# supranational/sppark

Measured on AMD Instinct MI355X. Metric: MSM points/sec (BLS12-381 G1, 2^26 points), higher is better.
Workload: dtype u32

## Files before the change

### sppark_amd/csrc/ec/xyzzx_dev.hpp

```cpp
#pragma once
#include "../ff/montx_dev.hpp"
#include "xyzz_dev.hpp"

namespace sppark_amd {

template<class FP> struct field_is_internal { static constexpr bool value = false; };
template<class P, int LB> struct field_is_internal<montx_dev<P, LB>> { static constexpr bool value = true; };
template<class FP> struct field_is_montx { static constexpr bool value = false; };
template<class P, int LB> struct field_is_montx<montx_dev<P, LB>> { static constexpr bool value = true; };

template<class P, int LB> struct affine_loader<montx_dev<P, LB>> {
    typedef montx_dev<P, LB> F;
    static constexpr unsigned RAW = 2 * F::NL * 4;
    static constexpr unsigned STRIDE = RAW <= 64 ? 64 : RAW <= 128 ? 128 : ((RAW + 15) / 16) * 16;
    struct raw_t {
        u32 w[(RAW + 15) / 16 * 4];
        SPPARK_DEVFN void landed() const
        {
#if defined(__HIP_DEVICE_COMPILE__)
            #pragma unroll
            for (unsigned i = 0; i < (RAW + 15) / 16 * 4; i++) asm volatile("" :: "v"(w[i]));
#endif
        }
    };
// ... 15 lines not shown
    }
    template<bool FLAGGED>
    SPPARK_DEVFN static affine_dev<F> load(const unsigned char* base, size_t idx, unsigned)
    {   return decode(load_raw(base, idx));   }
    template<bool FLAGGED>
    SPPARK_DEVFN static void convert(unsigned char* dst, const unsigned char* src, size_t idx, unsigned stride)
    {
        typedef mont_dev<P> S;
        u32 wx[S::N], wy[S::N];
        bool inf;
        if (!FLAGGED && (S::N % 2) == 0 && (stride & 15) == 0 && ((size_t)src & 15) == 0) {
            const uint4* q = reinterpret_cast<const uint4*>(src + idx * (size_t)stride);
            u32 w[2 * S::N];
            #pragma unroll
            for (int i = 0; i < S::N / 2; i++) { uint4 v = q[i]; w[4*i] = v.x; w[4*i+1] = v.y; w[4*i+2] = v.z; w[4*i+3] = v.w; }
            u32 any = 0;
            #pragma unroll
            for (int i = 0; i < S::N; i++) { wx[i] = w[i]; wy[i] = w[S::N + i]; any |= w[i] | w[S::N + i]; }
            inf = any == 0;
        } else {
            affine_dev<S> p = affine_loader<S>::template load<FLAGGED>(src, idx, stride);
            p.X.to_wire(wx); p.Y.to_wire(wy);
            inf = p.inf;
        }
        F x = F::from_std(wx), y = F::from_std(wy);
        u32 w[STRIDE / 4] = {};
        x.to_wire(w); y.to_wire(w + F::NL);
        if (inf) w[F::NL - 1] |= 0x80000000u;
        uint4* q = reinterpret_cast<uint4*>(dst + idx * (size_t)STRIDE);
        #pragma unroll
        for (unsigned i = 0; i < STRIDE / 16; i++) q[i] = make_uint4(w[4*i], w[4*i+1], w[4*i+2], w[4*i+3]);
    }
};

template<class P, int LB> struct xyzz_dev<montx_dev<P, LB>> {
    typedef montx_dev<P, LB> F;
    F X, Y, ZZZ, ZZ;
    static constexpr bool TIGHT = F::TIGHT;
    static constexpr int BX = TIGHT ? 1 : 6;
    static constexpr int BX2 = TIGHT ? 1 : 4;
    SPPARK_DEVFN static F keep_x(const F& x3) { if constexpr (TIGHT) return x3.norm(); else return x3; }
    SPPARK_DEVFN static F minus_y(const F& y) { if constexpr (TIGHT) return F::template neg<4, 2>(y); else return F::template neg<6, 4>(y); }

    SPPARK_DEVFN bool is_inf() const { return ZZ.limbs_all_zero(); }
    SPPARK_DEVFN void set_inf() { X = F::zero(); Y = F::zero(); ZZZ = F::zero(); ZZ = F::zero(); }

    SPPARK_DEVFN void set(const affine_dev<F>& p, bool negate)
    {
        if (p.inf) { set_inf(); return; }
        X = p.X; Y = negate ? F::template neg<3>(p.Y) : p.Y;
        ZZZ = F::one(); ZZ = F::one();
    }

    SPPARK_DEVFN void madd(const affine_dev<F>& p, bool negate)
    {
        if (p.inf) return;
        if (is_inf()) { set(p, negate); return; }

        F U2, S2;
        F::template mul2<true, true>(U2, S2, p.X, ZZ, p.Y, ZZZ);
        if (negate) S2 = F::template neg<3>(S2);
        F Pd = F::template sub<11, BX>(U2, X).norm();
        F Rd;
        if constexpr (TIGHT) Rd = F::template sub<4, 2>(S2, Y).norm(); else Rd = F::template sub<6, 4>(S2, Y).norm();

        if (!Pd.template is_zero_mod<13>()) {
            F PP, RR, PPP, Q;
            F::sqr2(PP, RR, Pd, Rd);
            F::template mul2<true, false>(PPP, Q, Pd, PP, X, PP);
            F T   = PPP + Q + Q;
            F X3  = keep_x(F::template sub<8, 3>(RR, T));
            F D   = F::template sub<11, BX>(Q, X3);
            F nY  = minus_y(Y);
            Y   = F::mul_add(D, Rd, nY, PPP);
            F::template mul2<true, true>(ZZ, ZZZ, ZZ, PP, ZZZ, PPP);
            X = X3;
        } else if (Rd.template is_zero_mod<9>()) {
            F y2 = negate ? F::template neg<3>(p.Y).norm() : p.Y;
            dbl_affine(p.X, y2);
        } else {
            set_inf();
        }
    }

    SPPARK_DEVFN void add(const xyzz_dev& q)
    {
        if (q.is_inf()) return;
        if (is_inf()) { *this = q; return; }

        F U1 = X * q.ZZ;
        F S1 = Y * q.ZZZ;
        F U2 = q.X * ZZ;
        F S2 = q.Y * ZZZ;
        F Pd = F::template sub<3>(U2, U1).norm();
        F Rd = F::template sub<3>(S2, S1).norm();

        if (!Pd.template is_zero_mod<5>()) {
            F PP  = Pd.sqr();
            F PPP = Pd * PP;
            F Q   = U1 * PP;
            F T   = PPP + Q + Q;
            F X3  = keep_x(F::template sub<8, 3>(Rd.sqr(), T));
            F D   = F::template sub<11, BX>(Q, X3);
            Y   = F::mul_add(D, Rd, F::template neg<3>(S1), PPP);
            ZZ  = (ZZ * PP) * q.ZZ;
            ZZZ = (ZZZ * PPP) * q.ZZZ;
            X = X3;
        } else if (Rd.template is_zero_mod<5>()) {
            xyzz_dev t = *this;
            dbl_outlined(t);
            *this = t;
        } else {
            set_inf();
        }
    }

    SPPARK_DEVFN void add_pairs(const xyzz_dev& q)
    {
        if (q.is_inf()) return;
        if (is_inf()) { *this = q; return; }
        F U1, S1, U2, S2;
        F::mul2(U1, S1, X, q.ZZ, Y, q.ZZZ);
        F::mul2(U2, S2, q.X, ZZ, q.Y, ZZZ);
        F Pd = F::template sub<3>(U2, U1).norm();
        F Rd = F::template sub<3>(S2, S1).norm();
        if (!Pd.template is_zero_mod<5>()) {
            F PP, RR, PPP, Q, t0, t1;
            F::sqr2(PP, RR, Pd, Rd);
            F::template mul2<true, true>(PPP, Q, Pd, PP, U1, PP);
            F T   = PPP + Q + Q;
            F X3  = keep_x(F::template sub<8, 3>(RR, T));
            F D   = F::template sub<11, BX>(Q, X3);
            Y   = F::mul_add(D, Rd, F::template neg<3>(S1), PPP);
            F::template mul2<true, true>(t0, t1, ZZ, PP, ZZZ, PPP);
// ... 102 lines not shown
```

### sppark_amd/csrc/ff/montx_blocks.hpp

```cpp
#pragma once
namespace sppark_amd {
#define MX_MAD(A, x, y) "v_mad_u64_u32 %[" #A "], vcc, %[" #x "], %[" #y "], %[" #A "]\n\t"
#define MX_SHR(A)       "v_lshrrev_b64 %[" #A "], %[LB], %[" #A "]\n\t"
#define MX_ADD(A, B)    "v_lshl_add_u64 %[" #A "], %[" #A "], 0, %[" #B "]\n\t"
#define MX_V(name, e)   [name] "v"(e)
#define MX_S(name, j)   [name] "s"(pl<F, j>)
#define MX_ASM(text, outs, ...) asm(text : outs : __VA_ARGS__, [LB] "n"(F::LIMB_BITS) : "vcc")
#define MX_ASM0(text, outs)     asm(text : outs : [LB] "n"(F::LIMB_BITS) : "vcc")
#define MX_ACC1 [A] "+v"(A)
#define MX_ACC2 [A0] "+v"(A0), [A1] "+v"(A1)
#define MX_ACCS [A] "+v"(A), [B] "+v"(B)
#define MX_I(j) (LO + j)
#define MX_J(j) (K - LO - j)
#define MX_MAX_TERMS 14
#define MX_T_AB1_1 MX_MAD(A, x0_0, y0_0)
#define MX_T_AB1_2 MX_T_AB1_1 MX_MAD(A, x0_1, y0_1)
#define MX_T_AB1_3 MX_T_AB1_2 MX_MAD(A, x0_2, y0_2)
#define MX_T_AB1_4 MX_T_AB1_3 MX_MAD(A, x0_3, y0_3)
#define MX_T_AB1_5 MX_T_AB1_4 MX_MAD(A, x0_4, y0_4)
#define MX_T_AB1_6 MX_T_AB1_5 MX_MAD(A, x0_5, y0_5)
#define MX_T_AB1_7 MX_T_AB1_6 MX_MAD(A, x0_6, y0_6)
#define MX_T_AB1_8 MX_T_AB1_7 MX_MAD(A, x0_7, y0_7)
#define MX_T_AB1_9 MX_T_AB1_8 MX_MAD(A, x0_8, y0_8)
#define MX_T_AB1_10 MX_T_AB1_9 MX_MAD(A, x0_9, y0_9)
#define MX_T_AB1_11 MX_T_AB1_10 MX_MAD(A, x0_10, y0_10)
#define MX_T_AB1_12 MX_T_AB1_11 MX_MAD(A, x0_11, y0_11)
#define MX_T_AB1_13 MX_T_AB1_12 MX_MAD(A, x0_12, y0_12)
#define MX_T_AB1_14 MX_T_AB1_13 MX_MAD(A, x0_13, y0_13)
#define MX_O_AB1_1 MX_V(x0_0, o.x0(MX_I(0), MX_J(0))), MX_V(y0_0, o.y0(MX_I(0), MX_J(0)))
#define MX_O_AB1_2 MX_O_AB1_1, MX_V(x0_1, o.x0(MX_I(1), MX_J(1))), MX_V(y0_1, o.y0(MX_I(1), MX_J(1)))
#define MX_O_AB1_3 MX_O_AB1_2, MX_V(x0_2, o.x0(MX_I(2), MX_J(2))), MX_V(y0_2, o.y0(MX_I(2), MX_J(2)))
#define MX_O_AB1_4 MX_O_AB1_3, MX_V(x0_3, o.x0(MX_I(3), MX_J(3))), MX_V(y0_3, o.y0(MX_I(3), MX_J(3)))
#define MX_O_AB1_5 MX_O_AB1_4, MX_V(x0_4, o.x0(MX_I(4), MX_J(4))), MX_V(y0_4, o.y0(MX_I(4), MX_J(4)))
#define MX_O_AB1_6 MX_O_AB1_5, MX_V(x0_5, o.x0(MX_I(5), MX_J(5))), MX_V(y0_5, o.y0(MX_I(5), MX_J(5)))
#define MX_O_AB1_7 MX_O_AB1_6, MX_V(x0_6, o.x0(MX_I(6), MX_J(6))), MX_V(y0_6, o.y0(MX_I(6), MX_J(6)))
#define MX_O_AB1_8 MX_O_AB1_7, MX_V(x0_7, o.x0(MX_I(7), MX_J(7))), MX_V(y0_7, o.y0(MX_I(7), MX_J(7)))
#define MX_O_AB1_9 MX_O_AB1_8, MX_V(x0_8, o.x0(MX_I(8), MX_J(8))), MX_V(y0_8, o.y0(MX_I(8), MX_J(8)))
#define MX_O_AB1_10 MX_O_AB1_9, MX_V(x0_9, o.x0(MX_I(9), MX_J(9))), MX_V(y0_9, o.y0(MX_I(9), MX_J(9)))
#define MX_O_AB1_11 MX_O_AB1_10, MX_V(x0_10, o.x0(MX_I(10), MX_J(10))), MX_V(y0_10, o.y0(MX_I(10), MX_J(10)))
#define MX_O_AB1_12 MX_O_AB1_11, MX_V(x0_11, o.x0(MX_I(11), MX_J(11))), MX_V(y0_11, o.y0(MX_I(11), MX_J(11)))
#define MX_O_AB1_13 MX_O_AB1_12, MX_V(x0_12, o.x0(MX_I(12), MX_J(12))), MX_V(y0_12, o.y0(MX_I(12), MX_J(12)))
#define MX_O_AB1_14 MX_O_AB1_13, MX_V(x0_13, o.x0(MX_I(13), MX_J(13))), MX_V(y0_13, o.y0(MX_I(13), MX_J(13)))
#define MX_T_MP1_1 MX_MAD(A, m0_0, p_0)
#define MX_T_MP1_2 MX_T_MP1_1 MX_MAD(A, m0_1, p_1)
#define MX_T_MP1_3 MX_T_MP1_2 MX_MAD(A, m0_2, p_2)
#define MX_T_MP1_4 MX_T_MP1_3 MX_MAD(A, m0_3, p_3)
#define MX_T_MP1_5 MX_T_MP1_4 MX_MAD(A, m0_4, p_4)
#define MX_T_MP1_6 MX_T_MP1_5 MX_MAD(A, m0_5, p_5)
#define MX_T_MP1_7 MX_T_MP1_6 MX_MAD(A, m0_6, p_6)
#define MX_T_MP1_8 MX_T_MP1_7 MX_MAD(A, m0_7, p_7)
#define MX_T_MP1_9 MX_T_MP1_8 MX_MAD(A, m0_8, p_8)
#define MX_T_MP1_10 MX_T_MP1_9 MX_MAD(A, m0_9, p_9)
#define MX_T_MP1_11 MX_T_MP1_10 MX_MAD(A, m0_10, p_10)
#define MX_T_MP1_12 MX_T_MP1_11 MX_MAD(A, m0_11, p_11)
#define MX_T_MP1_13 MX_T_MP1_12 MX_MAD(A, m0_12, p_12)
#define MX_T_MP1_14 MX_T_MP1_13 MX_MAD(A, m0_13, p_13)
#define MX_O_MP1_1 MX_V(m0_0, o.m0(MX_I(0))), MX_S(p_0, MX_J(0))
// ... 235 lines not shown
        else if constexpr (!CLOSE && NAB == 12 && NMP == 12) MX_ASM(MX_SHR(A0) MX_SHR(A1) MX_T_AB2_12(A0, A1) MX_T_MP2_12, MX_ACC2, MX_O_AB2_12, MX_O_MP2_12);
        else static_assert(K < 0, "no block of this shape");
#else
        if constexpr (CLOSE) { A0 += (u64)o.m0(K - 1) * F::mod_limb(0); A1 += (u64)o.m1(K - 1) * F::mod_limb(0); }
        if constexpr (K > 0) { A0 >>= F::LIMB_BITS; A1 >>= F::LIMB_BITS; }
        for (int j = 0; j < NAB; j++) { A0 += (u64)o.x0(MX_I(j), MX_J(j)) * o.y0(MX_I(j), MX_J(j)); A1 += (u64)o.x1(MX_I(j), MX_J(j)) * o.y1(MX_I(j), MX_J(j)); }
        for (int j = 0; j < NMP; j++) { A0 += (u64)o.m0(MX_I(j)) * F::mod_limb(MX_J(j)); A1 += (u64)o.m1(MX_I(j)) * F::mod_limb(MX_J(j)); }
#endif
    }
    template<class F, int K, class OPS> SPPARK_DEVFN static void col_sum(u64& A, const OPS& o)
    {
        MX_SHAPE;
        [[maybe_unused]] u64 B = 0;
#if defined(__HIP_DEVICE_COMPILE__)
        if constexpr (LAST) MX_ASM0(MX_SHR(A), MX_ACC1);
        else if constexpr (K == 0) { static_assert(NAB == 1 && NMP == 0, "shape"); asm(MX_T_AB2_1(A, B) MX_ADD(A, B) : MX_ACCS : MX_O_AB2_1 : "vcc"); }
        else if constexpr (CLOSE && NAB == 2 && NMP == 1) MX_ASM(MX_MAD(A, mc0, pc) MX_SHR(A) MX_T_AB2_2(A, B) MX_T_MPS_1 MX_ADD(A, B), MX_ACCS, MX_V(mc0, o.m0(K - 1)), MX_S(pc, 0), MX_O_AB2_2, MX_O_MP1_1);
        else if constexpr (CLOSE && NAB == 3 && NMP == 2) MX_ASM(MX_MAD(A, mc0, pc) MX_SHR(A) MX_T_AB2_3(A, B) MX_T_MPS_2 MX_ADD(A, B), MX_ACCS, MX_V(mc0, o.m0(K - 1)), MX_S(pc, 0), MX_O_AB2_3, MX_O_MP1_2);
        else if constexpr (CLOSE && NAB == 4 && NMP == 3) MX_ASM(MX_MAD(A, mc0, pc) MX_SHR(A) MX_T_AB2_4(A, B) MX_T_MPS_3 MX_ADD(A, B), MX_ACCS, MX_V(mc0, o.m0(K - 1)), MX_S(pc, 0), MX_O_AB2_4, MX_O_MP1_3);
        else if constexpr (CLOSE && NAB == 5 && NMP == 4) MX_ASM(MX_MAD(A, mc0, pc) MX_SHR(A) MX_T_AB2_5(A, B) MX_T_MPS_4 MX_ADD(A, B), MX_ACCS, MX_V(mc0, o.m0(K - 1)), MX_S(pc, 0), MX_O_AB2_5, MX_O_MP1_4);
        else if constexpr (CLOSE && NAB == 6 && NMP == 5) MX_ASM(MX_MAD(A, mc0, pc) MX_SHR(A) MX_T_AB2_6(A, B) MX_T_MPS_5 MX_ADD(A, B), MX_ACCS, MX_V(mc0, o.m0(K - 1)), MX_S(pc, 0), MX_O_AB2_6, MX_O_MP1_5);
        else if constexpr (CLOSE && NAB == 7 && NMP == 6) MX_ASM(MX_MAD(A, mc0, pc) MX_SHR(A) MX_T_AB2_7(A, B) MX_T_MPS_6 MX_ADD(A, B), MX_ACCS, MX_V(mc0, o.m0(K - 1)), MX_S(pc, 0), MX_O_AB2_7, MX_O_MP1_6);
        else if constexpr (CLOSE && NAB == 8 && NMP == 7) MX_ASM(MX_MAD(A, mc0, pc) MX_SHR(A) MX_T_AB2_8(A, B) MX_T_MPS_7 MX_ADD(A, B), MX_ACCS, MX_V(mc0, o.m0(K - 1)), MX_S(pc, 0), MX_O_AB2_8, MX_O_MP1_7);
        else if constexpr (CLOSE && NAB == 8 && NMP == 8) MX_ASM(MX_MAD(A, mc0, pc) MX_SHR(A) MX_T_AB2_8(A, B) MX_T_MPS_8 MX_ADD(A, B), MX_ACCS, MX_V(mc0, o.m0(K - 1)), MX_S(pc, 0), MX_O_AB2_8, MX_O_MP1_8);
        else if constexpr (CLOSE && NAB == 9 && NMP == 8) MX_ASM(MX_MAD(A, mc0, pc) MX_SHR(A) MX_T_AB2_9(A, B) MX_T_MPS_8 MX_ADD(A, B), MX_ACCS, MX_V(mc0, o.m0(K - 1)), MX_S(pc, 0), MX_O_AB2_9, MX_O_MP1_8);
        else if constexpr (CLOSE && NAB == 9 && NMP == 9) MX_ASM(MX_MAD(A, mc0, pc) MX_SHR(A) MX_T_AB2_9(A, B) MX_T_MPS_9 MX_ADD(A, B), MX_ACCS, MX_V(mc0, o.m0(K - 1)), MX_S(pc, 0), MX_O_AB2_9, MX_O_MP1_9);
        else if constexpr (CLOSE && NAB == 10 && NMP == 9) MX_ASM(MX_MAD(A, mc0, pc) MX_SHR(A) MX_T_AB2_10(A, B) MX_T_MPS_9 MX_ADD(A, B), MX_ACCS, MX_V(mc0, o.m0(K - 1)), MX_S(pc, 0), MX_O_AB2_10, MX_O_MP1_9);
        else if constexpr (CLOSE && NAB == 11 && NMP == 10) MX_ASM(MX_MAD(A, mc0, pc) MX_SHR(A) MX_T_AB2_11(A, B) MX_T_MPS_10 MX_ADD(A, B), MX_ACCS, MX_V(mc0, o.m0(K - 1)), MX_S(pc, 0), MX_O_AB2_11, MX_O_MP1_10);
        else if constexpr (CLOSE && NAB == 12 && NMP == 11) MX_ASM(MX_MAD(A, mc0, pc) MX_SHR(A) MX_T_AB2_12(A, B) MX_T_MPS_11 MX_ADD(A, B), MX_ACCS, MX_V(mc0, o.m0(K - 1)), MX_S(pc, 0), MX_O_AB2_12, MX_O_MP1_11);
        else if constexpr (CLOSE && NAB == 13 && NMP == 12) MX_ASM(MX_MAD(A, mc0, pc) MX_SHR(A) MX_T_AB2_13(A, B) MX_T_MPS_12 MX_ADD(A, B), MX_ACCS, MX_V(mc0, o.m0(K - 1)), MX_S(pc, 0), MX_O_AB2_13, MX_O_MP1_12);
        else if constexpr (CLOSE && NAB == 13 && NMP == 13) MX_ASM(MX_MAD(A, mc0, pc) MX_SHR(A) MX_T_AB2_13(A, B) MX_T_MPS_13 MX_ADD(A, B), MX_ACCS, MX_V(mc0, o.m0(K - 1)), MX_S(pc, 0), MX_O_AB2_13, MX_O_MP1_13);
        else if constexpr (CLOSE && NAB == 14 && NMP == 13) MX_ASM(MX_MAD(A, mc0, pc) MX_SHR(A) MX_T_AB2_14(A, B) MX_T_MPS_13 MX_ADD(A, B), MX_ACCS, MX_V(mc0, o.m0(K - 1)), MX_S(pc, 0), MX_O_AB2_14, MX_O_MP1_13);
        else if constexpr (!CLOSE && NAB == 1 && NMP == 1) MX_ASM(MX_SHR(A) MX_T_AB2_1(A, B) MX_T_MPS_1 MX_ADD(A, B), MX_ACCS, MX_O_AB2_1, MX_O_MP1_1);
        else if constexpr (!CLOSE && NAB == 2 && NMP == 2) MX_ASM(MX_SHR(A) MX_T_AB2_2(A, B) MX_T_MPS_2 MX_ADD(A, B), MX_ACCS, MX_O_AB2_2, MX_O_MP1_2);
        else if constexpr (!CLOSE && NAB == 3 && NMP == 3) MX_ASM(MX_SHR(A) MX_T_AB2_3(A, B) MX_T_MPS_3 MX_ADD(A, B), MX_ACCS, MX_O_AB2_3, MX_O_MP1_3);
        else if constexpr (!CLOSE && NAB == 4 && NMP == 4) MX_ASM(MX_SHR(A) MX_T_AB2_4(A, B) MX_T_MPS_4 MX_ADD(A, B), MX_ACCS, MX_O_AB2_4, MX_O_MP1_4);
        else if constexpr (!CLOSE && NAB == 5 && NMP == 5) MX_ASM(MX_SHR(A) MX_T_AB2_5(A, B) MX_T_MPS_5 MX_ADD(A, B), MX_ACCS, MX_O_AB2_5, MX_O_MP1_5);
        else if constexpr (!CLOSE && NAB == 6 && NMP == 6) MX_ASM(MX_SHR(A) MX_T_AB2_6(A, B) MX_T_MPS_6 MX_ADD(A, B), MX_ACCS, MX_O_AB2_6, MX_O_MP1_6);
        else if constexpr (!CLOSE && NAB == 7 && NMP == 7) MX_ASM(MX_SHR(A) MX_T_AB2_7(A, B) MX_T_MPS_7 MX_ADD(A, B), MX_ACCS, MX_O_AB2_7, MX_O_MP1_7);
        else if constexpr (!CLOSE && NAB == 8 && NMP == 8) MX_ASM(MX_SHR(A) MX_T_AB2_8(A, B) MX_T_MPS_8 MX_ADD(A, B), MX_ACCS, MX_O_AB2_8, MX_O_MP1_8);
        else if constexpr (!CLOSE && NAB == 9 && NMP == 9) MX_ASM(MX_SHR(A) MX_T_AB2_9(A, B) MX_T_MPS_9 MX_ADD(A, B), MX_ACCS, MX_O_AB2_9, MX_O_MP1_9);
        else if constexpr (!CLOSE && NAB == 10 && NMP == 10) MX_ASM(MX_SHR(A) MX_T_AB2_10(A, B) MX_T_MPS_10 MX_ADD(A, B), MX_ACCS, MX_O_AB2_10, MX_O_MP1_10);
        else if constexpr (!CLOSE && NAB == 11 && NMP == 11) MX_ASM(MX_SHR(A) MX_T_AB2_11(A, B) MX_T_MPS_11 MX_ADD(A, B), MX_ACCS, MX_O_AB2_11, MX_O_MP1_11);
        else if constexpr (!CLOSE && NAB == 12 && NMP == 12) MX_ASM(MX_SHR(A) MX_T_AB2_12(A, B) MX_T_MPS_12 MX_ADD(A, B), MX_ACCS, MX_O_AB2_12, MX_O_MP1_12);
        else static_assert(K < 0, "no block of this shape");
#else
        if constexpr (CLOSE) A += (u64)o.m0(K - 1) * F::mod_limb(0);
        if constexpr (K > 0) A >>= F::LIMB_BITS;
        for (int j = 0; j < NAB; j++) { A += (u64)o.x0(MX_I(j), MX_J(j)) * o.y0(MX_I(j), MX_J(j)); B += (u64)o.x1(MX_I(j), MX_J(j)) * o.y1(MX_I(j), MX_J(j)); }
        for (int j = 0; j < NMP; j++) (j & 1 ? B : A) += (u64)o.m0(MX_I(j)) * F::mod_limb(MX_J(j));
        A += B;
#endif
    }
};
#undef MX_MAD
#undef MX_SHR
#undef MX_ADD
#undef MX_V
#undef MX_S
#undef MX_ASM
#undef MX_ASM0
#undef MX_ACC1
#undef MX_ACC2
#undef MX_ACCS
#undef MX_I
#undef MX_J
#undef MX_SHAPE
#undef MX_O_AB1_1
#undef MX_O_AB1_10
#undef MX_O_AB1_11
#undef MX_O_AB1_12
#undef MX_O_AB1_13
#undef MX_O_AB1_14
#undef MX_O_AB1_2
#undef MX_O_AB1_3
#undef MX_O_AB1_4
#undef MX_O_AB1_5
#undef MX_O_AB1_6
#undef MX_O_AB1_7
#undef MX_O_AB1_8
#undef MX_O_AB1_9
#undef MX_O_AB2_1
#undef MX_O_AB2_10
#undef MX_O_AB2_11
#undef MX_O_AB2_12
#undef MX_O_AB2_13
#undef MX_O_AB2_14
#undef MX_O_AB2_2
#undef MX_O_AB2_3
#undef MX_O_AB2_4
#undef MX_O_AB2_5
#undef MX_O_AB2_6
#undef MX_O_AB2_7
#undef MX_O_AB2_8
#undef MX_O_AB2_9
#undef MX_O_MP1_1
#undef MX_O_MP1_10
#undef MX_O_MP1_11
#undef MX_O_MP1_12
#undef MX_O_MP1_13
#undef MX_O_MP1_14
#undef MX_O_MP1_2
#undef MX_O_MP1_3
#undef MX_O_MP1_4
#undef MX_O_MP1_5
#undef MX_O_MP1_6
#undef MX_O_MP1_7
#undef MX_O_MP1_8
#undef MX_O_MP1_9
#undef MX_O_MP2_1
// ... 86 lines not shown
```

### sppark_amd/csrc/ff/montx_dev.hpp

```cpp
#pragma once
#include "mont_dev.hpp"
#include "montx_blocks.hpp"
#include <utility>

namespace sppark_amd {


#if defined(SPPARK_HOST_EMULATION) && defined(SPPARK_TRACK_BOUNDS)
extern "C" void sppark_bound_violation(const char* what, double got, double limit);
#endif
template<class P, int LB> struct montx_dev {
    static constexpr int NW = P::N;
    static constexpr int HEAD = LB <= 28 ? 8 : 6;
    static constexpr int NL = (P::NBITS + HEAD + LB - 1) / LB;
    static constexpr int CAP = 1 << (32 - LB);
    static constexpr int FAT_L = 1 << (31 - LB);
    static constexpr bool TIGHT = LB > 28;
    static constexpr bool FAT_M_OK = (double)NL * (4294967296.0 * (double)(1ull << LB) + (double)(1ull << LB) * (double)(1ull << LB))
                                     + 68719476736.0 < 18446744073709551616.0;
    static constexpr int MA_A0 = TIGHT ? 3 : FAT_L, MA_A1 = TIGHT ? 3 : 6;
    static constexpr int SQR_L = TIGHT ? 2 : 4;
    static constexpr int N = NL;
    static constexpr int LIMB_BITS = LB;
    typedef montx_blocks blk;
// ... 169 lines not shown
    }

    SPPARK_DEVFN static montx_dev from_wire(const u32* w)
    {   montx_dev r; for (int j = 0; j < NL; j++) r.l[j] = w[j]; return r;   }
    SPPARK_DEVFN void to_wire(u32* w) const { for (int j = 0; j < NL; j++) w[j] = l[j]; }

    SPPARK_DEVFN static montx_dev zero() { montx_dev r; for (int j = 0; j < NL; j++) r.l[j] = 0; SPPARK_BND(r.bnd_set(0.0, 0.0);) return r; }
    SPPARK_DEVFN bool limbs_all_zero() const
    {   u32 acc = l[0]; for (int j = 1; j < NL; j++) acc |= l[j]; return acc == 0;   }

    SPPARK_DEVFN montx_dev norm() const
    {
        montx_dev r; u32 c = 0;
        #pragma unroll
        for (int j = 0; j < NL - 1; j++) { u32 v = l[j] + c; r.l[j] = v & MASK; c = v >> LB; }
        r.l[NL - 1] = l[NL - 1] + c;
        SPPARK_BND(bnd_known("norm: operand"); bnd(bl <= (double)(CAP - 1), "norm: limbs", bl, (double)(CAP - 1)); r.bnd_set(bv, bl < 1.0 ? bl : 1.0);)
        return r;
    }

    SPPARK_DEVFN friend montx_dev operator+(const montx_dev& a, const montx_dev& b)
    {
        montx_dev r;
        #pragma unroll
        for (int j = 0; j < NL; j++) r.l[j] = a.l[j] + b.l[j];
        SPPARK_BND(a.bnd_known("+: left"); b.bnd_known("+: right"); r.bnd_set(a.bv + b.bv, a.bl + b.bl); bnd(r.bl < (double)CAP, "+: limbs wrap", r.bl, (double)CAP);)
        return r;
    }

    template<int K, int B = 1> SPPARK_DEVFN static montx_dev sub(const montx_dev& a, const montx_dev& b)
    {
        montx_dev r;
        #pragma unroll
        for (int j = 0; j < NL; j++) r.l[j] = a.l[j] + (fat_tab<K, B>::T.l[j] - b.l[j]);
        SPPARK_BND(a.bnd_known("sub: minuend"); b.bnd_known("sub: subtrahend");
                   bnd(b.bv <= (double)(K - 1), "sub<K>: subtrahend < (K-1) p", b.bv, (double)(K - 1));
                   bnd(b.bl <= (double)B, "sub<K,B>: subtrahend's limbs <= B 2^LB", b.bl, (double)B);
                   r.bnd_set(a.bv + (double)K, a.bl + (double)(B + 1));
                   bnd(r.bl < (double)CAP, "sub: limbs wrap", r.bl, (double)CAP);)
        return r;
    }
    template<int K, int B = 1> SPPARK_DEVFN static montx_dev neg(const montx_dev& b)
    {
        montx_dev r;
        #pragma unroll
        for (int j = 0; j < NL; j++) r.l[j] = fat_tab<K, B>::T.l[j] - b.l[j];
        SPPARK_BND(b.bnd_known("neg: operand");
                   bnd(b.bv <= (double)(K - 1), "neg<K>: operand < (K-1) p", b.bv, (double)(K - 1));
                   bnd(b.bl <= (double)B, "neg<K,B>: operand's limbs <= B 2^LB", b.bl, (double)B);
                   r.bnd_set((double)K, (double)(B + 1));)
        return r;
    }


    SPPARK_DEVFN friend montx_dev operator*(const montx_dev& a, const montx_dev& b)
    {
        constexpr u32 PINV = P::M0 & MASK;
        u32 m[NL];
        montx_dev r;
        u64 A = 0;
        for_columns([&] SPPARK_COLUMN(kc, k)
            blk::template col1<montx_dev, k>(A, blk::mul_ops{a.l, b.l, nullptr, nullptr, m, nullptr});
            if constexpr (k < NL) m[k] = ((u32)A * PINV) & MASK;
            else        r.l[k - NL] = (u32)A & MASK;
        });
        SPPARK_BND(a.bnd_known("*: left"); b.bnd_known("*: right");
                   bnd(b.bl <= 1.0, "*: right operand normalised", b.bl, 1.0);
                   bnd(a.bl <= FAT_LEFT + 1e-6, "*: left operand's limbs < 2^31", a.bl, FAT_LEFT);
                   r.bnd_set(a.bv * b.bv / rho() + 1.0, 1.0);)
        return r;
    }
    template<bool FAT_M> SPPARK_DEVFN static u32 quotient_digit(u64 A, int k)
    {
        constexpr u32 PINV = P::M0 & MASK;
        if (FAT_M && FAT_M_OK && k < NL - 1) return (u32)A * (u32)P::M0;
        return ((u32)A * PINV) & MASK;
    }

    template<bool NORM0 = false, bool NORM1 = false>
    SPPARK_DEVFN static void mul2(montx_dev& r0, montx_dev& r1,
                                  const montx_dev& a0, const montx_dev& b0,
                                  const montx_dev& a1, const montx_dev& b1)
    {
        u32 m0[NL], m1[NL];
        u64 A0 = 0, A1 = 0;
        for_columns([&] SPPARK_COLUMN(kc, k)
            blk::template col2<montx_dev, k>(A0, A1, blk::mul_ops{a0.l, b0.l, a1.l, b1.l, m0, m1});
            if constexpr (k < NL) { m0[k] = quotient_digit<NORM0>(A0, k); m1[k] = quotient_digit<NORM1>(A1, k); }
            else        { r0.l[k - NL] = (u32)A0 & MASK; r1.l[k - NL] = (u32)A1 & MASK; }
        });
        SPPARK_BND(a0.bnd_known("mul2: a0"); b0.bnd_known("mul2: b0"); a1.bnd_known("mul2: a1"); b1.bnd_known("mul2: b1");
                   bnd(b0.bl <= 1.0 && b1.bl <= 1.0, "mul2: right operands normalised", b0.bl > b1.bl ? b0.bl : b1.bl, 1.0);
                   bnd(a0.bl <= (NORM0 ? 1.0 : FAT_LEFT) + 1e-6, NORM0 ? "mul2<NORM0>: a0 normalised" : "mul2: a0's limbs < 2^31", a0.bl, NORM0 ? 1.0 : FAT_LEFT);
                   bnd(a1.bl <= (NORM1 ? 1.0 : FAT_LEFT) + 1e-6, NORM1 ? "mul2<NORM1>: a1 normalised" : "mul2: a1's limbs < 2^31", a1.bl, NORM1 ? 1.0 : FAT_LEFT);
                   r0.bnd_set(a0.bv * b0.bv / rho() + 1.0 + (NORM0 ? 1e-6 : 0.0), 1.0);
                   r1.bnd_set(a1.bv * b1.bv / rho() + 1.0 + (NORM1 ? 1e-6 : 0.0), 1.0);)
    }
    SPPARK_DEVFN static montx_dev mul_add(const montx_dev& a0, const montx_dev& b0,
                                          const montx_dev& a1, const montx_dev& b1)
    {
        static_assert((double)NL * ((double)MA_A0 + (double)MA_A1 + 1.0) * (double)(1ull << LB) * (double)(1ull << LB) + 68719476736.0
                      < 18446744073709551616.0, "a column of two products must fit the 64-bit accumulator");
        constexpr u32 PINV = P::M0 & MASK;
        u32 m[NL];
        montx_dev r;
        u64 A = 0;
        for_columns([&] SPPARK_COLUMN(kc, k)
            blk::template col_sum<montx_dev, k>(A, blk::mul_ops{a0.l, b0.l, a1.l, b1.l, m, nullptr});
            if constexpr (k < NL) m[k] = ((u32)A * PINV) & MASK;
            else        r.l[k - NL] = (u32)A & MASK;
        });
        SPPARK_BND(a0.bnd_known("mul_add: a0"); b0.bnd_known("mul_add: b0"); a1.bnd_known("mul_add: a1"); b1.bnd_known("mul_add: b1");
                   bnd(b0.bl <= 1.0 && b1.bl <= 1.0, "mul_add: right operands normalised", b0.bl > b1.bl ? b0.bl : b1.bl, 1.0);
                   bnd(a0.bl <= (double)MA_A0 + 1e-6, "mul_add: a0's limbs <= MA_A0 2^LB", a0.bl, (double)MA_A0);
                   bnd(a1.bl <= (double)MA_A1, "mul_add: a1's limbs <= MA_A1 2^LB", a1.bl, (double)MA_A1);
                   r.bnd_set((a0.bv * b0.bv + a1.bv * b1.bv) / rho() + 1.0, 1.0);)
        return r;
    }

    SPPARK_DEVFN static void sqr2(montx_dev& r0, montx_dev& r1, const montx_dev& a0, const montx_dev& a1)
    {
        u32 m0[NL], m1[NL], d0[NL], d1[NL];
        #pragma unroll
        for (int j = 0; j < NL; j++) { d0[j] = a0.l[j] << 1; d1[j] = a1.l[j] << 1; }
        u64 A0 = 0, A1 = 0;
        for_columns([&] SPPARK_COLUMN(kc, k)
            blk::template col2<montx_dev, k>(A0, A1, blk::sqr_ops{a0.l, d0, a1.l, d1, m0, m1});
            if constexpr (k < NL) { m0[k] = quotient_digit<true>(A0, k); m1[k] = quotient_digit<true>(A1, k); }
            else        { r0.l[k - NL] = (u32)A0 & MASK; r1.l[k - NL] = (u32)A1 & MASK; }
        });
        SPPARK_BND(a0.bnd_known("sqr2: a0"); a1.bnd_known("sqr2: a1");
                   bnd(a0.bl <= 1.0 && a1.bl <= 1.0, "sqr2: operands normalised", a0.bl > a1.bl ? a0.bl : a1.bl, 1.0);
                   r0.bnd_set(a0.bv * a0.bv / rho() + 1.0 + 1e-6, 1.0); r1.bnd_set(a1.bv * a1.bv / rho() + 1.0 + 1e-6, 1.0);)
    }

    SPPARK_DEVFN montx_dev sqr() const
    {
        static_assert(((double)(NL / 2) * 2.0 * SQR_L * SQR_L + (double)(SQR_L * SQR_L) + (double)NL) * (double)(1ull << LB) * (double)(1ull << LB)
                      + 68719476736.0 < 18446744073709551616.0, "a column of a square of limbs <= SQR_L 2^LB must fit the 64-bit accumulator");
        constexpr u32 PINV = P::M0 & MASK;
        u32 m[NL], d[NL];
        #pragma unroll
        for (int j = 0; j < NL; j++) d[j] = l[j] << 1;
        montx_dev r;
        u64 A = 0;
        for_columns([&] SPPARK_COLUMN(kc, k)
            blk::template col1<montx_dev, k>(A, blk::sqr_ops{l, d, nullptr, nullptr, m, nullptr});
            if constexpr (k < NL) m[k] = ((u32)A * PINV) & MASK;
            else        r.l[k - NL] = (u32)A & MASK;
        });
        SPPARK_BND(bnd_known("sqr: operand"); bnd(bl <= (double)SQR_L, "sqr: limbs <= SQR_L 2^LB", bl, (double)SQR_L); r.bnd_set(bv * bv / rho() + 1.0, 1.0);)
        return r;
    }

    SPPARK_DEVFN montx_dev inverse() const
    {
        montx_dev r = one();
        bool started = false;
        #pragma unroll 1
        for (int w = NW - 1; w >= 0; w--) {
            u32 e = 0, borrow = 2;
            for (int k = 0; k <= w; k++) { e = P::MOD[k] - borrow; borrow = P::MOD[k] < borrow ? 1u : 0u; }
            #pragma unroll 1
            for (int b = 31; b >= 0; b--) {
                if (started) r = r.sqr();
                if ((e >> b) & 1u) { r = started ? r * *this : *this; started = true; }
            }
        }
        return r;
    }

    template<int KMAX> SPPARK_DEVFN bool is_zero_mod() const
    {
        SPPARK_BND(bnd_known("is_zero_mod: operand"); bnd(bl <= 1.0, "is_zero_mod: normalised", bl, 1.0);
                   bnd(bv <= (double)KMAX, "is_zero_mod<KMAX>: value < KMAX p", bv, (double)KMAX);)
        bool maybe = false;
        #pragma unroll
        for (int kk = 0; kk < KMAX; kk++) maybe |= (l[0] == multiples_tab<KMAX>::T.l[kk][0]);
        if (!maybe) return false;
        bool hit = false;
        #pragma unroll 1
        for (int k = 0; k < KMAX; k++) {
            u32 diff = 0;
            #pragma unroll
            for (int j = 0; j < NL; j++) diff |= multiples_tab<KMAX>::T.l[k][j] ^ l[j];
            hit |= diff == 0;
        }
        return hit;
    }
};

}
```

### sppark_amd/csrc/msm/msm_kernels.hpp

```cpp
#pragma once
#include "../ec/xyzz_dev.hpp"
#include "../ec/xyzzx_dev.hpp"

namespace sppark_amd {

static constexpr u32 KEY_NONE = 0xffffffffu;


__host__ __device__ inline unsigned window_len(unsigned w, unsigned nwins, unsigned nbits)
{   return nbits / nwins + (w < nbits % nwins ? 1u : 0u);   }

template<class LimbFn>
SPPARK_DEVFN void recode_digits(u32* digits, size_t n, size_t i, LimbFn limb, bool flip,
                                unsigned nwins, unsigned nbits, unsigned w_begin = 0, unsigned w_count = ~0u)
{
    u32 carry = 0;
    const unsigned w_end = w_count > nwins - w_begin ? nwins : w_begin + w_count;
    for (unsigned w = 0, bit = 0; w < w_end; w++) {
        const unsigned len = window_len(w, nwins, nbits);
        const u32 half = 1u << (len - 1), full = 1u << len, mask = full - 1;
        const unsigned li = bit >> 5, sh = bit & 31;
        bit += len;
        u64 two = limb(li) | ((u64)limb(li + 1) << 32);
        u32 d = ((u32)(two >> sh) & mask) + carry;
// ... 23 lines not shown
    flip = bw != 0;
    return FR::select(flip, neg, s);
}

template<class FR>
__global__ __launch_bounds__(256)
void k_breakdown(u32* __restrict__ digits, const u32* __restrict__ scalars,
                 unsigned n, unsigned nwins, unsigned nbits, int mont, unsigned w_begin, unsigned w_count)
{
    constexpr int N = FR::N;
    __shared__ u32 limbs[N + 2][256];
    const unsigned tid = threadIdx.x;
    for (unsigned i = blockIdx.x * 256 + tid; i < n; i += gridDim.x * 256) {
        bool flip;
        FR s = load_scalar_abs<FR>(scalars, i, mont, flip);
        #pragma unroll
        for (int k = 0; k < N; k++) limbs[k][tid] = s.v[k];
        limbs[N][tid] = 0; limbs[N + 1][tid] = 0;
        recode_digits(digits, n, i, [&](unsigned k) { return limbs[k][tid]; }, flip, nwins, nbits, w_begin, w_count);
    }
}

template<class FP, bool ON> struct gather_raw { struct type {}; };
template<class FP> struct gather_raw<FP, true> { typedef typename affine_loader<FP>::raw_t type; };

template<class FP, bool FLAGGED>
SPPARK_DEVFN void accumulate_chunk(xyzz_mem<FP::N>* buckets, u32* rec_key, xyzz_mem<FP::N>* rec_pt,
                                   const unsigned char* points, unsigned stride,
                                   const u32* sorted, const u32* off,
                                   unsigned n, unsigned NB, unsigned L, unsigned chunks_per_win,
                                   unsigned chunk, unsigned w_local, unsigned w_base = 0)
{
    if (chunk >= chunks_per_win) return;
    const unsigned w = w_base + w_local;
    const size_t rec0 = ((size_t)w * chunks_per_win + chunk) * 2;
    const u32* o = off + (size_t)w_local * (NB + 1);
    const unsigned total = o[NB];
    unsigned p = chunk * L;
    if (p >= total) { rec_key[rec0] = KEY_NONE; rec_key[rec0 + 1] = KEY_NONE; return; }
    const unsigned end = total < p + L ? total : p + L;

    unsigned lo = 0, hi = NB;
    while (hi - lo > 1) {
        unsigned mid = (lo + hi) >> 1;
        if (o[mid] <= p) lo = mid; else hi = mid;
    }
    unsigned b = lo, next = o[b + 1], next2 = o[b + 2 < NB ? b + 2 : NB];

    const u32* src = sorted + (size_t)w_local * n;
    xyzz_dev<FP> acc;
    bool first_run = true;
    u32 slot0_key = KEY_NONE;

    u32 e = src[p];
    affine_dev<FP> pt = load_affine<FP, FLAGGED>(points, e & 0x7fffffffu, stride);
    acc.set(pt, e >> 31);
    constexpr bool PREFETCH = field_is_montx<FP>::value;
    u32 e_next = 0, e_next2 = 0;
    typename gather_raw<FP, PREFETCH>::type raw_next = {};
    const unsigned last = end - 1;
    if constexpr (PREFETCH) {
        e_next = src[p + 1 < last ? p + 1 : last];
        raw_next = affine_loader<FP>::load_raw(points, e_next & 0x7fffffffu);
        e_next2 = src[p + 2 < last ? p + 2 : last];
    }
    if constexpr (PREFETCH) raw_next.landed();
    for (p++; p < end; p++) {
        if constexpr (PREFETCH) {
            e = e_next; pt = affine_loader<FP>::decode(raw_next);
        } else {
            e = src[p];
            pt = load_affine<FP, FLAGGED>(points, e & 0x7fffffffu, stride);
        }
        if (p == next) {
            const u32 key = w * NB + b;
            if (first_run) { acc.store(&rec_pt[rec0]); slot0_key = key; first_run = false; }
            else           acc.store(&buckets[key]);
            b++; next = next2;
            if (p == next) do { b++; next = o[b + 1]; } while (p == next);
            next2 = o[b + 2 < NB ? b + 2 : NB];
            acc.set_inf();
        }
        if constexpr (PREFETCH) {
            e_next = e_next2;
            raw_next = affine_loader<FP>::load_raw(points, e_next & 0x7fffffffu);
            e_next2 = src[p + 2 < last ? p + 2 : last];
        }
        acc.madd(pt, e >> 31);
    }
    const u32 key = w * NB + b;
    if (first_run) { acc.store(&rec_pt[rec0]); rec_key[rec0] = key; rec_key[rec0 + 1] = KEY_NONE; }
    else           { acc.store(&rec_pt[rec0 + 1]); rec_key[rec0] = slot0_key; rec_key[rec0 + 1] = key; }
}

#ifndef SPPARK_G2_TWO_WAVES_MAX_N
# define SPPARK_G2_TWO_WAVES_MAX_N 20
#endif
template<class FP, bool FLAGGED>
__global__ __launch_bounds__(256, (field_is_internal<FP>::value && FP::N <= 10) ? 3 : (field_is_internal<FP>::value && FP::N <= SPPARK_G2_TWO_WAVES_MAX_N) ? 2 : 1)
void k_accumulate(xyzz_mem<FP::N>* __restrict__ buckets,
                  u32* __restrict__ rec_key, xyzz_mem<FP::N>* __restrict__ rec_pt,
                  const unsigned char* __restrict__ points, unsigned stride,
                  const u32* __restrict__ sorted, const u32* __restrict__ off,
                  unsigned n, unsigned NB, unsigned L, unsigned chunks_per_win, unsigned w_base)
{
    accumulate_chunk<FP, FLAGGED>(buckets, rec_key, rec_pt, points, stride, sorted, off, n, NB, L,
                                  chunks_per_win, blockIdx.x * blockDim.x + threadIdx.x, blockIdx.y, w_base);
}

template<class FP, bool FLAGGED>
SPPARK_DEVFN void bitmap_accumulate_item(u32* rec_key, xyzz_mem<FP::N>* rec_pt,
                                         const unsigned char* points, unsigned stride, unsigned npoints,
                                         const u32* bitmap, const u32* refmap, unsigned span_words, size_t t)
{
    const size_t nwords = ((size_t)npoints + 31) / 32;
    const size_t w0 = t * span_words;
    if (w0 >= nwords) return;
    xyzz_dev<FP> acc; acc.set_inf();
    for (size_t w = w0; w < w0 + span_words && w < nwords; w++) {
        u32 bits = bitmap[w], refs = refmap ? refmap[w] : 0;
        bits ^= refs; refs &= bits;
        if (w == nwords - 1 && (npoints & 31)) bits &= (1u << (npoints & 31)) - 1;
        while (bits) {
            const unsigned k = __builtin_ctz(bits);
            bits &= bits - 1;
            affine_dev<FP> p = load_affine<FP, FLAGGED>(points, w * 32 + k, stride);
            acc.madd(p, (refs >> k) & 1);
        }
    }
    acc.store(&rec_pt[t]); rec_key[t] = 0;
}
template<class FP, bool FLAGGED>
__global__ __launch_bounds__(256)
void k_bitmap_accumulate(u32* __restrict__ rec_key, xyzz_mem<FP::N>* __restrict__ rec_pt,
                         const unsigned char* __restrict__ points, unsigned stride, unsigned npoints,
                         const u32* __restrict__ bitmap, const u32* __restrict__ refmap, unsigned span_words)
{
    bitmap_accumulate_item<FP, FLAGGED>(rec_key, rec_pt, points, stride, npoints, bitmap, refmap, span_words,
                                        (size_t)blockIdx.x * blockDim.x + threadIdx.x);
}

static constexpr unsigned JOIN_WALK = 8;
template<class FP> SPPARK_DEVFN void bucket_add(xyzz_dev<FP>& a, const xyzz_dev<FP>& b);
template<class FP> SPPARK_DEVFN void bucket_add_fast(xyzz_dev<FP>& a, const xyzz_dev<FP>& b);

template<class FP>
SPPARK_DEVFN void join_runs_item(xyzz_mem<FP::N>* buckets, u32* out_key, const u32* in_key,
                                 const xyzz_mem<FP::N>* in_pt, unsigned nrec, u32* any_long, size_t t)
{
    size_t job_h[2], job_e[2]; u32 job_k[2]; unsigned njobs = 0;
    for (unsigned s = 0; s < 2; s++) {
        if (t == 0 && s == 0) continue;
        const size_t q = 2 * t - 1 + s;
        if (q >= nrec) break;
        const u32 k = in_key[q];
        if (k == KEY_NONE) { out_key[q] = KEY_NONE; continue; }
        size_t h = q; bool is_long = false;
        for (size_t i = q, none = 0; i-- > 0;) {
            const u32 ki = in_key[i];
            if (ki == KEY_NONE) { if (++none == 2) break; continue; }
            none = 0;
            if (ki != k) break;
            h = i;
            if (q - h > JOIN_WALK) { is_long = true; break; }
        }
        size_t e = h;
        if (!is_long) {
            bool ended = false;
            size_t i = h + 1;
            for (unsigned none = 0; i < nrec && i <= h + JOIN_WALK; i++) {
                const u32 ki = in_key[i];
                if (ki == KEY_NONE) { if (++none == 2) { ended = true; break; } continue; }
                none = 0;
                if (ki != k) { ended = true; break; }
                e = i;
            }
            if (i >= nrec) ended = true;
            is_long = !ended;
        }
        if (is_long) { out_key[q] = k; *any_long = 1; continue; }
        out_key[q] = KEY_NONE;
        if (q == h) { job_h[njobs] = h; job_e[njobs] = e; job_k[njobs] = k; njobs++; }
// ... 431 lines not shown
```

Measured before the change: 523.3 million.

## Fuse mixed-add subtractions into Montgomery mul2 and track accumulator infinity in a flag

Adds a mul2_sub primitive that folds the Pd/Rd subtractions (U2-X, S2-Y) into the final columns of the paired Montgomery multiplication through a new asm column block, and replaces the branchy negate with a conditional negation on the affine Y. The accumulator's point-at-infinity state becomes a register flag instead of a scan of ZZ's limbs, so resetting to infinity no longer writes four field elements. is_zero_mod now uses a multiplicative precheck on the low limb in place of a loop over a table of multiples. These changes aim to cut instruction count in the hot bucket-accumulation madd, at the cost of more template/asm surface and tight lazy-reduction bound requirements.

Result: no change. 524.4 million (median of 6 runs) (+0.2%).

```diff
diff --git a/sppark_amd/csrc/ec/xyzzx_dev.hpp b/sppark_amd/csrc/ec/xyzzx_dev.hpp
--- a/sppark_amd/csrc/ec/xyzzx_dev.hpp
+++ b/sppark_amd/csrc/ec/xyzzx_dev.hpp
@@ -91,17 +91,17 @@
         ZZZ = F::one(); ZZ = F::one();
     }
 
-    SPPARK_DEVFN void madd(const affine_dev<F>& p, bool negate)
+    SPPARK_DEVFN void madd(const affine_dev<F>& p, bool negate) { bool unused = false; madd_any<false>(p, negate, unused); }
+    SPPARK_DEVFN void madd(const affine_dev<F>& p, bool negate, bool& inf) { madd_any<true>(p, negate, inf); }
+
+    template<bool FLAG> SPPARK_DEVFN void madd_any(const affine_dev<F>& p, bool negate, bool& inf)
     {
         if (p.inf) return;
-        if (is_inf()) { set(p, negate); return; }
-
-        F U2, S2;
-        F::template mul2<true, true>(U2, S2, p.X, ZZ, p.Y, ZZZ);
-        if (negate) S2 = F::template neg<3>(S2);
-        F Pd = F::template sub<11, BX>(U2, X).norm();
-        F Rd;
-        if constexpr (TIGHT) Rd = F::template sub<4, 2>(S2, Y).norm(); else Rd = F::template sub<6, 4>(S2, Y).norm();
+        if (FLAG ? inf : is_inf()) { set(p, negate); inf = false; return; }
+
+        F ys = F::template cneg<3>(p.Y, negate);
+        F Pd, Rd;
+        F::template mul2_sub<true, false, 11, BX, TIGHT ? 4 : 6, TIGHT ? 2 : 4>(Pd, Rd, p.X, ZZ, ys, ZZZ, X, Y);
 
         if (!Pd.template is_zero_mod<13>()) {
             F PP, RR, PPP, Q;
@@ -115,10 +115,9 @@
             F::template mul2<true, true>(ZZ, ZZZ, ZZ, PP, ZZZ, PPP);
             X = X3;
         } else if (Rd.template is_zero_mod<9>()) {
-            F y2 = negate ? F::template neg<3>(p.Y).norm() : p.Y;
-            dbl_affine(p.X, y2);
-        } else {
-            set_inf();
+            dbl_affine(p.X, ys.norm());
+        } else {
+            if constexpr (FLAG) inf = true; else set_inf();
         }
     }
 
diff --git a/sppark_amd/csrc/ff/montx_blocks.hpp b/sppark_amd/csrc/ff/montx_blocks.hpp
--- a/sppark_amd/csrc/ff/montx_blocks.hpp
+++ b/sppark_amd/csrc/ff/montx_blocks.hpp
@@ -3,6 +3,7 @@
 #define MX_MAD(A, x, y) "v_mad_u64_u32 %[" #A "], vcc, %[" #x "], %[" #y "], %[" #A "]\n\t"
 #define MX_SHR(A)       "v_lshrrev_b64 %[" #A "], %[LB], %[" #A "]\n\t"
 #define MX_ADD(A, B)    "v_lshl_add_u64 %[" #A "], %[" #A "], 0, %[" #B "]\n\t"
+#define MX_ONE(A, c)    "v_mad_i64_i32 %[" #A "], vcc, %[" #c "], 1, %[" #A "]\n\t"
 #define MX_V(name, e)   [name] "v"(e)
 #define MX_S(name, j)   [name] "s"(pl<F, j>)
 #define MX_ASM(text, outs, ...) asm(text : outs : __VA_ARGS__, [LB] "n"(F::LIMB_BITS) : "vcc")
@@ -344,10 +345,40 @@
         A += B;
 #endif
     }
+    template<class F, int K, class OPS> SPPARK_DEVFN static void col2_sub(u64& A0, u64& A1, const OPS& o, u32 c0, u32 c1)
+    {
+        MX_SHAPE;
+        static_assert(K >= NL && !LAST, "an output column but the last");
+#if defined(__HIP_DEVICE_COMPILE__)
+        if constexpr (CLOSE && NAB == 8 && NMP == 8) MX_ASM(MX_MAD(A0, mc0, pc) MX_MAD(A1, mc1, pc) MX_SHR(A0) MX_SHR(A1) MX_T_AB2_8(A0, A1) MX_T_MP2_8 MX_ONE(A0, c0) MX_ONE(A1, c1), MX_ACC2, MX_V(mc0, o.m0(K - 1)), MX_S(pc, 0), MX_V(mc1, o.m1(K - 1)), MX_O_AB2_8, MX_O_MP2_8, MX_V(c0, c0), MX_V(c1, c1));
+        else if constexpr (CLOSE && NAB == 9 && NMP == 9) MX_ASM(MX_MAD(A0, mc0, pc) MX_MAD(A1, mc1, pc) MX_SHR(A0) MX_SHR(A1) MX_T_AB2_9(A0, A1) MX_T_MP2_9 MX_ONE(A0, c0) MX_ONE(A1, c1), MX_ACC2, MX_V(mc0, o.m0(K - 1)), MX_S(pc, 0), MX_V(mc1, o.m1(K - 1)), MX_O_AB2_9, MX_O_MP2_9, MX_V(c0, c0), MX_V(c1, c1));
+        else if constexpr (CLOSE && NAB == 13 && NMP == 13) MX_ASM(MX_MAD(A0, mc0, pc) MX_MAD(A1, mc1, pc) MX_SHR(A0) MX_SHR(A1) MX_T_AB2_13(A0, A1) MX_T_MP2_13 MX_ONE(A0, c0) MX_ONE(A1, c1), MX_ACC2, MX_V(mc0, o.m0(K - 1)), MX_S(pc, 0), MX_V(mc1, o.m1(K - 1)), MX_O_AB2_13, MX_O_MP2_13, MX_V(c0, c0), MX_V(c1, c1));
+        else if constexpr (!CLOSE && NAB == 1 && NMP == 1) MX_ASM(MX_SHR(A0) MX_SHR(A1) MX_T_AB2_1(A0, A1) MX_T_MP2_1 MX_ONE(A0, c0) MX_ONE(A1, c1), MX_ACC2, MX_O_AB2_1, MX_O_MP2_1, MX_V(c0, c0), MX_V(c1, c1));
+        else if constexpr (!CLOSE && NAB == 2 && NMP == 2) MX_ASM(MX_SHR(A0) MX_SHR(A1) MX_T_AB2_2(A0, A1) MX_T_MP2_2 MX_ONE(A0, c0) MX_ONE(A1, c1), MX_ACC2, MX_O_AB2_2, MX_O_MP2_2, MX_V(c0, c0), MX_V(c1, c1));
+        else if constexpr (!CLOSE && NAB == 3 && NMP == 3) MX_ASM(MX_SHR(A0) MX_SHR(A1) MX_T_AB2_3(A0, A1) MX_T_MP2_3 MX_ONE(A0, c0) MX_ONE(A1, c1), MX_ACC2, MX_O_AB2_3, MX_O_MP2_3, MX_V(c0, c0), MX_V(c1, c1));
+        else if constexpr (!CLOSE && NAB == 4 && NMP == 4) MX_ASM(MX_SHR(A0) MX_SHR(A1) MX_T_AB2_4(A0, A1) MX_T_MP2_4 MX_ONE(A0, c0) MX_ONE(A1, c1), MX_ACC2, MX_O_AB2_4, MX_O_MP2_4, MX_V(c0, c0), MX_V(c1, c1));
+        else if constexpr (!CLOSE && NAB == 5 && NMP == 5) MX_ASM(MX_SHR(A0) MX_SHR(A1) MX_T_AB2_5(A0, A1) MX_T_MP2_5 MX_ONE(A0, c0) MX_ONE(A1, c1), MX_ACC2, MX_O_AB2_5, MX_O_MP2_5, MX_V(c0, c0), MX_V(c1, c1));
+        else if constexpr (!CLOSE && NAB == 6 && NMP == 6) MX_ASM(MX_SHR(A0) MX_SHR(A1) MX_T_AB2_6(A0, A1) MX_T_MP2_6 MX_ONE(A0, c0) MX_ONE(A1, c1), MX_ACC2, MX_O_AB2_6, MX_O_MP2_6, MX_V(c0, c0), MX_V(c1, c1));
+        else if constexpr (!CLOSE && NAB == 7 && NMP == 7) MX_ASM(MX_SHR(A0) MX_SHR(A1) MX_T_AB2_7(A0, A1) MX_T_MP2_7 MX_ONE(A0, c0) MX_ONE(A1, c1), MX_ACC2, MX_O_AB2_7, MX_O_MP2_7, MX_V(c0, c0), MX_V(c1, c1));
+        else if constexpr (!CLOSE && NAB == 8 && NMP == 8) MX_ASM(MX_SHR(A0) MX_SHR(A1) MX_T_AB2_8(A0, A1) MX_T_MP2_8 MX_ONE(A0, c0) MX_ONE(A1, c1), MX_ACC2, MX_O_AB2_8, MX_O_MP2_8, MX_V(c0, c0), MX_V(c1, c1));
+        else if constexpr (!CLOSE && NAB == 9 && NMP == 9) MX_ASM(MX_SHR(A0) MX_SHR(A1) MX_T_AB2_9(A0, A1) MX_T_MP2_9 MX_ONE(A0, c0) MX_ONE(A1, c1), MX_ACC2, MX_O_AB2_9, MX_O_MP2_9, MX_V(c0, c0), MX_V(c1, c1));
+        else if constexpr (!CLOSE && NAB == 10 && NMP == 10) MX_ASM(MX_SHR(A0) MX_SHR(A1) MX_T_AB2_10(A0, A1) MX_T_MP2_10 MX_ONE(A0, c0) MX_ONE(A1, c1), MX_ACC2, MX_O_AB2_10, MX_O_MP2_10, MX_V(c0, c0), MX_V(c1, c1));
+        else if constexpr (!CLOSE && NAB == 11 && NMP == 11) MX_ASM(MX_SHR(A0) MX_SHR(A1) MX_T_AB2_11(A0, A1) MX_T_MP2_11 MX_ONE(A0, c0) MX_ONE(A1, c1), MX_ACC2, MX_O_AB2_11, MX_O_MP2_11, MX_V(c0, c0), MX_V(c1, c1));
+        else if constexpr (!CLOSE && NAB == 12 && NMP == 12) MX_ASM(MX_SHR(A0) MX_SHR(A1) MX_T_AB2_12(A0, A1) MX_T_MP2_12 MX_ONE(A0, c0) MX_ONE(A1, c1), MX_ACC2, MX_O_AB2_12, MX_O_MP2_12, MX_V(c0, c0), MX_V(c1, c1));
+        else static_assert(K < 0, "no block of this shape");
+#else
+        if constexpr (CLOSE) { A0 += (u64)o.m0(K - 1) * F::mod_limb(0); A1 += (u64)o.m1(K - 1) * F::mod_limb(0); }
+        A0 >>= F::LIMB_BITS; A1 >>= F::LIMB_BITS;
+        for (int j = 0; j < NAB; j++) { A0 += (u64)o.x0(MX_I(j), MX_J(j)) * o.y0(MX_I(j), MX_J(j)); A1 += (u64)o.x1(MX_I(j), MX_J(j)) * o.y1(MX_I(j), MX_J(j)); }
+        for (int j = 0; j < NMP; j++) { A0 += (u64)o.m0(MX_I(j)) * F::mod_limb(MX_J(j)); A1 += (u64)o.m1(MX_I(j)) * F::mod_limb(MX_J(j)); }
+        A0 += c0; A1 += c1;
+#endif
+    }
 };
 #undef MX_MAD
 #undef MX_SHR
 #undef MX_ADD
+#undef MX_ONE
 #undef MX_V
 #undef MX_S
 #undef MX_ASM
diff --git a/sppark_amd/csrc/ff/montx_dev.hpp b/sppark_amd/csrc/ff/montx_dev.hpp
--- a/sppark_amd/csrc/ff/montx_dev.hpp
+++ b/sppark_amd/csrc/ff/montx_dev.hpp
@@ -245,6 +245,18 @@
         return r;
     }
 
+    template<int K, int B = 1> SPPARK_DEVFN static montx_dev cneg(const montx_dev& b, bool flag)
+    {
+        montx_dev r;
+        #pragma unroll
+        for (int j = 0; j < NL; j++) r.l[j] = flag ? fat_tab<K, B>::T.l[j] - b.l[j] : b.l[j];
+        SPPARK_BND(b.bnd_known("cneg: operand");
+                   bnd(b.bv <= (double)(K - 1), "cneg<K>: operand < (K-1) p", b.bv, (double)(K - 1));
+                   bnd(b.bl <= (double)B, "cneg<K,B>: operand's limbs <= B 2^LB", b.bl, (double)B);
+                   r.bnd_set((double)K > b.bv ? (double)K : b.bv, (double)(B + 1));)
+        return r;
+    }
+
 
     SPPARK_DEVFN friend montx_dev operator*(const montx_dev& a, const montx_dev& b)
     {
@@ -288,6 +300,43 @@
                    bnd(a1.bl <= (NORM1 ? 1.0 : FAT_LEFT) + 1e-6, NORM1 ? "mul2<NORM1>: a1 normalised" : "mul2: a1's limbs < 2^31", a1.bl, NORM1 ? 1.0 : FAT_LEFT);
                    r0.bnd_set(a0.bv * b0.bv / rho() + 1.0 + (NORM0 ? 1e-6 : 0.0), 1.0);
                    r1.bnd_set(a1.bv * b1.bv / rho() + 1.0 + (NORM1 ? 1e-6 : 0.0), 1.0);)
+    }
+    template<bool NORM0, bool NORM1, int K0, int B0, int K1, int B1>
+    SPPARK_DEVFN static void mul2_sub(montx_dev& r0, montx_dev& r1,
+                                      const montx_dev& a0, const montx_dev& b0,
+                                      const montx_dev& a1, const montx_dev& b1,
+                                      const montx_dev& s0, const montx_dev& s1)
+    {
+        static_assert(((u64)(B0 + 1) << LB) <= (1ull << 31) && ((u64)(B1 + 1) << LB) <= (1ull << 31), "the lazy term is below 2^31");
+        u32 m0[NL], m1[NL];
+        u64 A0 = 0, A1 = 0;
+        for_columns([&] SPPARK_COLUMN(kc, k)
+            if constexpr (k < NL) {
+                blk::template col2<montx_dev, k>(A0, A1, blk::mul_ops{a0.l, b0.l, a1.l, b1.l, m0, m1});
+                m0[k] = quotient_digit<NORM0>(A0, k); m1[k] = quotient_digit<NORM1>(A1, k);
+            } else {
+                const u32 c0 = fat_tab<K0, B0>::T.l[k - NL] - s0.l[k - NL], c1 = fat_tab<K1, B1>::T.l[k - NL] - s1.l[k - NL];
+                if constexpr (k < 2 * NL - 1) {
+                    blk::template col2_sub<montx_dev, k>(A0, A1, blk::mul_ops{a0.l, b0.l, a1.l, b1.l, m0, m1}, c0, c1);
+                    r0.l[k - NL] = (u32)A0 & MASK; r1.l[k - NL] = (u32)A1 & MASK;
+                } else {
+                    blk::template col2<montx_dev, k>(A0, A1, blk::mul_ops{a0.l, b0.l, a1.l, b1.l, m0, m1});
+                    r0.l[k - NL] = (u32)A0 + c0; r1.l[k - NL] = (u32)A1 + c1;
+                }
+            }
+        });
+        SPPARK_BND(a0.bnd_known("mul2_sub: a0"); b0.bnd_known("mul2_sub: b0"); a1.bnd_known("mul2_sub: a1"); b1.bnd_known("mul2_sub: b1");
+                   s0.bnd_known("mul2_sub: s0"); s1.bnd_known("mul2_sub: s1");
+                   bnd(b0.bl <= 1.0 && b1.bl <= 1.0, "mul2_sub: right operands normalised", b0.bl > b1.bl ? b0.bl : b1.bl, 1.0);
+                   bnd(a0.bl <= (NORM0 ? 1.0 : FAT_LEFT) + 1e-6, NORM0 ? "mul2_sub<NORM0>: a0 normalised" : "mul2_sub: a0's limbs < 2^31", a0.bl, NORM0 ? 1.0 : FAT_LEFT);
+                   bnd(a1.bl <= (NORM1 ? 1.0 : FAT_LEFT) + 1e-6, NORM1 ? "mul2_sub<NORM1>: a1 normalised" : "mul2_sub: a1's limbs < 2^31", a1.bl, NORM1 ? 1.0 : FAT_LEFT);
+                   bnd(s0.bv <= (double)(K0 - 1), "mul2_sub<K0>: subtrahend < (K-1) p", s0.bv, (double)(K0 - 1));
+                   bnd(s1.bv <= (double)(K1 - 1), "mul2_sub<K1>: subtrahend < (K-1) p", s1.bv, (double)(K1 - 1));
+                   bnd(s0.bl <= (double)B0, "mul2_sub<K0,B0>: subtrahend's limbs <= B 2^LB", s0.bl, (double)B0);
+                   bnd(s1.bl <= (double)B1, "mul2_sub<K1,B1>: subtrahend's limbs <= B 2^LB", s1.bl, (double)B1);
+                   bnd((double)(B0 + 2) <= (double)(CAP - 1) && (double)(B1 + 2) <= (double)(CAP - 1), "mul2_sub: limbs wrap", (double)((B0 > B1 ? B0 : B1) + 2), (double)(CAP - 1));
+                   r0.bnd_set(a0.bv * b0.bv / rho() + 1.0 + (NORM0 ? 1e-6 : 0.0) + (double)K0, 1.0);
+                   r1.bnd_set(a1.bv * b1.bv / rho() + 1.0 + (NORM1 ? 1e-6 : 0.0) + (double)K1, 1.0);)
     }
     SPPARK_DEVFN static montx_dev mul_add(const montx_dev& a0, const montx_dev& b0,
                                           const montx_dev& a1, const montx_dev& b1)
@@ -367,10 +416,8 @@
     {
         SPPARK_BND(bnd_known("is_zero_mod: operand"); bnd(bl <= 1.0, "is_zero_mod: normalised", bl, 1.0);
                    bnd(bv <= (double)KMAX, "is_zero_mod<KMAX>: value < KMAX p", bv, (double)KMAX);)
-        bool maybe = false;
-        #pragma unroll
-        for (int kk = 0; kk < KMAX; kk++) maybe |= (l[0] == multiples_tab<KMAX>::T.l[kk][0]);
-        if (!maybe) return false;
+        constexpr u32 PREC = (0u - (P::M0 & MASK)) & MASK;
+        if (((l[0] * PREC) & MASK) >= (u32)KMAX) return false;
         bool hit = false;
         #pragma unroll 1
         for (int k = 0; k < KMAX; k++) {
diff --git a/sppark_amd/csrc/msm/msm_kernels.hpp b/sppark_amd/csrc/msm/msm_kernels.hpp
--- a/sppark_amd/csrc/msm/msm_kernels.hpp
+++ b/sppark_amd/csrc/msm/msm_kernels.hpp
@@ -99,9 +99,12 @@
     bool first_run = true;
     u32 slot0_key = KEY_NONE;
 
+    constexpr bool INF_FLAG = field_is_montx<FP>::value;
+    bool acc_inf = true;
+
     u32 e = src[p];
     affine_dev<FP> pt = load_affine<FP, FLAGGED>(points, e & 0x7fffffffu, stride);
-    acc.set(pt, e >> 31);
+    if constexpr (INF_FLAG) acc.madd(pt, e >> 31, acc_inf); else acc.set(pt, e >> 31);
     constexpr bool PREFETCH = field_is_montx<FP>::value;
     u32 e_next = 0, e_next2 = 0;
     typename gather_raw<FP, PREFETCH>::type raw_next = {};
@@ -121,21 +124,23 @@
         }
         if (p == next) {
             const u32 key = w * NB + b;
+            if constexpr (INF_FLAG) if (acc_inf) acc.set_inf();
             if (first_run) { acc.store(&rec_pt[rec0]); slot0_key = key; first_run = false; }
             else           acc.store(&buckets[key]);
             b++; next = next2;
             if (p == next) do { b++; next = o[b + 1]; } while (p == next);
-            next2 = o[b + 2 < NB ? b + 2 : NB];
-            acc.set_inf();
-        }
+            if constexpr (INF_FLAG) acc_inf = true; else acc.set_inf();
+        }
+        next2 = o[b + 2 < NB ? b + 2 : NB];
         if constexpr (PREFETCH) {
             e_next = e_next2;
             raw_next = affine_loader<FP>::load_raw(points, e_next & 0x7fffffffu);
             e_next2 = src[p + 2 < last ? p + 2 : last];
         }
-        acc.madd(pt, e >> 31);
+        if constexpr (INF_FLAG) acc.madd(pt, e >> 31, acc_inf); else acc.madd(pt, e >> 31);
     }
     const u32 key = w * NB + b;
+    if constexpr (INF_FLAG) if (acc_inf) acc.set_inf();
     if (first_run) { acc.store(&rec_pt[rec0]); rec_key[rec0] = key; rec_key[rec0 + 1] = KEY_NONE; }
     else           { acc.store(&rec_pt[rec0 + 1]); rec_key[rec0] = slot0_key; rec_key[rec0 + 1] = key; }
 }
@@ -163,7 +168,10 @@
     const size_t nwords = ((size_t)npoints + 31) / 32;
     const size_t w0 = t * span_words;
     if (w0 >= nwords) return;
-    xyzz_dev<FP> acc; acc.set_inf();
+    constexpr bool INF_FLAG = field_is_montx<FP>::value;
+    xyzz_dev<FP> acc;
+    bool acc_inf = true;
+    if constexpr (!INF_FLAG) acc.set_inf();
     for (size_t w = w0; w < w0 + span_words && w < nwords; w++) {
         u32 bits = bitmap[w], refs = refmap ? refmap[w] : 0;
         bits ^= refs; refs &= bits;
@@ -172,9 +180,10 @@
             const unsigned k = __builtin_ctz(bits);
             bits &= bits - 1;
             affine_dev<FP> p = load_affine<FP, FLAGGED>(points, w * 32 + k, stride);
-            acc.madd(p, (refs >> k) & 1);
-        }
-    }
+            if constexpr (INF_FLAG) acc.madd(p, (refs >> k) & 1, acc_inf); else acc.madd(p, (refs >> k) & 1);
+        }
+    }
+    if constexpr (INF_FLAG) if (acc_inf) acc.set_inf();
     acc.store(&rec_pt[t]); rec_key[t] = 0;
 }
 template<class FP, bool FLAGGED>
```
